# risingwavelabs/risingwave

Measured on NVIDIA H100. Metric: Nexmark q7/q8-shaped streaming HashJoin input rows/s, higher is better.
Workload: dtype int64

## Files before the change

__graft_entry__.py:

```python
import os
import subprocess
import sys

ROOT = os.path.dirname(os.path.abspath(__file__))
CSRC = os.path.join(ROOT, "risingwave_b200", "csrc")
BUILD = os.path.join(ROOT, "build")
LIB = os.path.join(ROOT, "risingwave_b200", "librwgpu.so")
NVCC = os.environ.get("NVCC", "/usr/local/cuda/bin/nvcc")
NVCC_FLAGS = ["-gencode", "arch=compute_90a,code=sm_90a", "-lineinfo", "-O3", "-std=c++17",
              "-Xcompiler", "-fPIC", "-Xcompiler", "-Wall"]
SOURCES = ["api.cu", "agg.cu", "join.cu", "shuffle.cu", "chain.cu"]


def _newer(target, deps):
    if not os.path.exists(target):
        return True
    t = os.path.getmtime(target)
    return any(os.path.getmtime(d) > t for d in deps)


def build_e2e_caller() -> str:
    os.makedirs(BUILD, exist_ok=True)
    e2e_src = os.path.join(ROOT, "tools", "e2e_caller.cc")
    e2e_bin = os.path.join(BUILD, "e2e_caller")
    if _newer(e2e_bin, [e2e_src, os.path.join(ROOT, "include", "rwgpu.h"), LIB]):
        subprocess.check_call(["g++", "-std=c++17", "-O2", "-Wall", "-I" + os.path.join(ROOT, "include"), "-I/usr/local/cuda/include", e2e_src,
                               "-o", e2e_bin, "-L" + os.path.join(ROOT, "risingwave_b200"), "-lrwgpu", "-L/usr/local/cuda/lib64", "-lcudart",
                               "-Wl,-rpath,$ORIGIN/../risingwave_b200", "-Wl,-rpath,/usr/local/cuda/lib64"])
    return e2e_bin


def build(verbose: bool = False) -> None:
    os.makedirs(BUILD, exist_ok=True)
    headers = [os.path.join(CSRC, f) for f in os.listdir(CSRC) if f.endswith((".cuh", ".h"))]
    headers.append(os.path.join(ROOT, "include", "rwgpu.h"))
    objs = []
    for src in SOURCES:
        s = os.path.join(CSRC, src)
        o = os.path.join(BUILD, src.replace(".cu", ".o"))
        objs.append(o)
        if _newer(o, [s] + headers):
            cmd = [NVCC] + NVCC_FLAGS + (["-Xptxas", "-v"] if verbose else []) + ["-c", s, "-o", o]
            subprocess.check_call(cmd)
    if _newer(LIB, objs):
        subprocess.check_call([NVCC] + NVCC_FLAGS[:2] + ["-shared", "-o", LIB] + objs + ["-lcudart"])
    subprocess.check_call(["make", "-s", "-C", os.path.join(ROOT, "oracle")])
    kat_src = os.path.join(ROOT, "tests", "cpp", "test_executor_kats.cc")
    kat_bin = os.path.join(BUILD, "test_executor_kats")
    if _newer(kat_bin, [kat_src, os.path.join(ROOT, "include", "rwgpu_executor.hpp"), LIB]):
        subprocess.check_call(["g++", "-std=c++17", "-O1", "-Wall", "-I" + os.path.join(ROOT, "include"), kat_src, "-o", kat_bin,
                               "-L" + os.path.join(ROOT, "risingwave_b200"), "-lrwgpu", "-Wl,-rpath,$ORIGIN/../risingwave_b200"])
    wm_src = os.path.join(ROOT, "tests", "cpp", "test_watermarks.cc")
    wm_bin = os.path.join(BUILD, "test_watermarks")
    if _newer(wm_bin, [wm_src, os.path.join(ROOT, "include", "rwgpu_executor.hpp"), LIB]):
        subprocess.check_call(["g++", "-std=c++17", "-O1", "-Wall", "-I" + os.path.join(ROOT, "include"), wm_src, "-o", wm_bin,
                               "-L" + os.path.join(ROOT, "risingwave_b200"), "-lrwgpu", "-Wl,-rpath,$ORIGIN/../risingwave_b200"])
    build_e2e_caller()
    sys.path.insert(0, ROOT)
    import risingwave_b200
    from risingwave_b200 import abi
    lib = abi.load_library()
    for sym in abi.ABI_SYMBOLS:
        getattr(lib, sym)


def smoke() -> None:
    sys.path.insert(0, ROOT)
    sys.path.insert(0, os.path.join(ROOT, "tests"))
    import ctypes
    import numpy as np
    from risingwave_b200.executor import Backend
    from risingwave_b200.stream_chunk import net_multiset
    import helpers
    cuda = Backend.cuda()
    oracle = Backend(ctypes.CDLL(os.path.join(ROOT, "oracle", "_build", "liboracle.so")), "rwo_")
    rng = np.random.default_rng(0)
    from risingwave_b200 import abi
    cfg = {"schema": "III", "group_keys": [0], "agg_calls": ["(count:int8)", "(sum:int8 $1:int8)", "(max:int8 $2:int8)"],
           "append_only": True, "row_count_index": 0}
    outs = []
    for be in (cuda, oracle):
        tx, ex = helpers.make_agg(be, cfg)
        res = []
        r2 = np.random.default_rng(1)
        for epoch in range(2):
            ex.apply_chunk(helpers.rand_chunk(r2, 4096, [abi.T_INT64] * 3, key_cols=(0,), key_range=300))
            res.append(net_multiset(ex.flush_data(epoch + 1)))
        outs.append(res)
    assert outs[0] == outs[1], "HashAgg smoke: CUDA result differs from oracle"
    print("smoke: HashAgg parity ok")
    try:
        kat = [k for k in helpers.load_golden("hash_join_kats.json") if k["name"] == "test_streaming_hash_inner_join"][0]
        helpers.run_join_kat(cuda, kat, exact=False)
        print("smoke: HashJoin golden ok")
    except abi.RwError as e:
        if e.code != abi.RW_ERR_UNSUPPORTED:
            raise
        print("smoke: HashJoin not built yet")


if __name__ == "__main__":
    build(verbose="-v" in sys.argv)
    print("build ok:", LIB)
```

risingwave_b200/csrc/join.cu:

```cuda
#include <algorithm>
#include <chrono>
#include <cstdio>
#include <cstdlib>
#include <memory>
#include <mutex>
#include <thread>

#include <cub/device/device_radix_sort.cuh>
#include <cub/device/device_scan.cuh>

#include "common.cuh"

namespace rw {

#define J_EMPTY 0x8000000000000000ull
#define J_NIL 0x7fffffffu
#define J_DEAD 0x80000000u
#define J_MAX_OUT (2 * RW_MAX_COLS)
#define J_HDR 16
#define W_EMPTY 0x7fffffffull
#define W_COUNT_ONE (1ull << 33)
#define W_IL_LIVE (1ull << 31)
#define W_IL_DEAD (2ull << 31)
#define W_IL_MASK (3ull << 31)
__device__ __host__ __forceinline__ uint32_t W_head(uint64_t W) { return (uint32_t)(W & 0x7fffffffull); }
__device__ __host__ __forceinline__ uint32_t W_istate(uint64_t W) { return (uint32_t)((W >> 31) & 3ull); }
__device__ __host__ __forceinline__ uint32_t W_count(uint64_t W) { return (uint32_t)(W >> 33); }

#define JERR_DOUBLE_DELETE 1u
#define JERR_OUT_CAPACITY 2u
#define JERR_APPEND_ONLY_MULTI 4u
#define JERR_STORE_CAPACITY 8u
#define JERR_BAD_COUNT 16u

struct JoinPlanDev {
  int T;
  int n_keys;
  int key_col[2][RW_MAX_KEYS];
  int null_safe[RW_MAX_KEYS];
  int n_cols[2];
  int col_type[2][RW_MAX_COLS];
  int col_width[2][RW_MAX_COLS];
  int col_off[2][RW_MAX_COLS];
  int stride[2];
  int bhdr;
  int bstride[2];
  int n_pk[2];
  int pk_col[2][RW_MAX_COLS];
  int n_out;
  int out_type[J_MAX_OUT];
  int out_width[J_MAX_OUT];
  int n_map[2];
  int map_in[2][J_MAX_OUT];
  int map_out[2][J_MAX_OUT];
  int need_degree[2];
  int append_only_optimize;
  int cond_cmp, cond_lhs, cond_rhs;
  int single_key, KW, SW;
  int strict;
};

struct JoinSideDev {
  uint8_t* recs;
  uint8_t* buckets;
  uint64_t cap;
  int stride;
  int bstride;
};

struct JoinStatus {
  unsigned long long out_rows;
  unsigned long long n_store;
  unsigned long long n_del;
  unsigned long long null_mask;
  unsigned long long n_keys[2];
  unsigned int err;
  unsigned int pad;
  unsigned long long n_in;
  unsigned long long log_next[2];
  unsigned long long n_dead[2];
  unsigned long long n_defer;
};

struct JoinOutDev {
  uint8_t* ops;
  uint8_t* vis;
  void* col[J_MAX_OUT];
  uint8_t* valid[J_MAX_OUT];
  int64_t capacity;
  const uint8_t* heap[2];
};

__device__ __host__ __forceinline__ bool jt_is_outer_side(int T, int S) { return T == RW_JOIN_FULL_OUTER || (T == RW_JOIN_LEFT_OUTER && S == 0) || (T == RW_JOIN_RIGHT_OUTER && S == 1); }
__device__ __host__ __forceinline__ bool jt_outer_side_null(int T, int S) { return T == RW_JOIN_FULL_OUTER || (T == RW_JOIN_LEFT_OUTER && S == 1) || (T == RW_JOIN_RIGHT_OUTER && S == 0); }
__device__ __host__ __forceinline__ bool jt_forward_exactly_once(int T, int S) { return ((T == RW_JOIN_LEFT_SEMI || T == RW_JOIN_LEFT_ANTI) && S == 0) || ((T == RW_JOIN_RIGHT_SEMI || T == RW_JOIN_RIGHT_ANTI) && S == 1); }
__device__ __host__ __forceinline__ bool jt_only_forward_matched_side(int T, int S) { return ((T == RW_JOIN_LEFT_SEMI || T == RW_JOIN_LEFT_ANTI) && S == 1) || ((T == RW_JOIN_RIGHT_SEMI || T == RW_JOIN_RIGHT_ANTI) && S == 0); }
__device__ __host__ __forceinline__ bool jt_is_semi(int T) { return T == RW_JOIN_LEFT_SEMI || T == RW_JOIN_RIGHT_SEMI; }
__device__ __host__ __forceinline__ bool jt_is_anti(int T) { return T == RW_JOIN_LEFT_ANTI || T == RW_JOIN_RIGHT_ANTI; }
__device__ __host__ __forceinline__ bool jt_forward_if_not_matched(int T, int S) { return (jt_is_anti(T) && jt_forward_exactly_once(T, S)) || jt_is_outer_side(T, S); }

struct RecHdr {
  uint32_t link, nullmask, seq, degree;
};
__device__ __forceinline__ uint8_t* rec_ptr(const JoinSideDev& s, uint32_t row) { return s.recs + (uint64_t)row * s.stride; }
__device__ __forceinline__ RecHdr* rec_hdr(const JoinSideDev& s, uint32_t row) { return (RecHdr*)rec_ptr(s, row); }

__device__ __forceinline__ uint64_t rec_key_word(const uint8_t* rec, int off, int width, int type) {
  ColRef cr;
  cr.data = rec + off;
  cr.valid_bits = nullptr;
  cr.valid_bytes = nullptr;
  cr.type = type;
  cr.width = width;
  return load_key_word(cr, 0);
}

__device__ __forceinline__ void prefetch_l2(const void* ptr) { asm volatile("prefetch.global.L2 [%0];" ::"l"(ptr)); }

__device__ __forceinline__ void copy_bytes(void* dst, const void* src, int width) {
  switch (width) {
    case 1: *(uint8_t*)dst = *(const uint8_t*)src; break;
    case 2: *(uint16_t*)dst = *(const uint16_t*)src; break;
    case 4: *(uint32_t*)dst = *(const uint32_t*)src; break;
    case 8: *(uint64_t*)dst = *(const uint64_t*)src; break;
    default: *(ulonglong2*)dst = *(const ulonglong2*)src; break;
  }
}

__device__ __forceinline__ bool chunk_key(const JoinPlanDev* p, int S, const DevChunk& ch, int64_t r, uint64_t* kw,
                                          uint32_t* nm) {
  uint32_t m = 0;
  bool never = false;
  for (int k = 0; k < p->n_keys; k++) {
    const ColRef& c = ch.cols[p->key_col[S][k]];
    if (col_is_null(c, r)) {
      m |= 1u << k;
      kw[k] = 0;
      if (!p->null_safe[k]) never = true;
    } else {
      kw[k] = load_key_word(c, r);
    }
  }
  *nm = m;
  return never;
}

__device__ __forceinline__ uint64_t key_hash(const JoinPlanDev* p, const uint64_t* kw, uint32_t nm) {
  uint64_t h = 0x9e3779b97f4a7c15ull ^ nm;
  for (int k = 0; k < p->n_keys; k++) h = mix64(h ^ kw[k]) + 0x9e3779b97f4a7c15ull;
  return h;
}

__device__ __forceinline__ uint64_t home64(uint64_t key, uint64_t mask) { return mix64(key) & mask & ~1ull; }

__device__ __forceinline__ uint8_t* bkt(const JoinSideDev& s, int64_t b) { return s.buckets + (uint64_t)b * s.bstride; }
__device__ __forceinline__ unsigned long long* bkt_W(const JoinSideDev& s, const JoinPlanDev* p, int64_t b) {
  return (unsigned long long*)(bkt(s, b) + p->KW * 8);
}
__device__ __forceinline__ uint8_t* bkt_inline(const JoinSideDev& s, const JoinPlanDev* p, int64_t b) { return bkt(s, b) + p->bhdr; }

__device__ __forceinline__ bool cas128(void* addr, ulonglong2 expect, ulonglong2 desired, ulonglong2* found) {
  unsigned long long o0, o1;
  asm volatile(
      "{\n .reg .b128 c, d, o;\n mov.b128 c, {%2, %3};\n mov.b128 d, {%4, %5};\n atom.global.cas.b128 o, [%6], c, d;\n mov.b128 {%0, %1}, o;\n}"
      : "=l"(o0), "=l"(o1)
      : "l"(expect.x), "l"(expect.y), "l"(desired.x), "l"(desired.y), "l"(addr)
      : "memory");
  found->x = o0;
  found->y = o1;
  return o0 == expect.x && o1 == expect.y;
}

__device__ __forceinline__ bool w_claim_inline(unsigned long long* Wp) {
  unsigned long long cur = __ldcg(Wp);
  while (W_istate(cur) != 1u) {
    const unsigned long long nw = ((cur & ~W_IL_MASK) | W_IL_LIVE) + W_COUNT_ONE;
    const unsigned long long old = atomicCAS(Wp, cur, nw);
    if (old == cur) return true;
    cur = old;
  }
  return false;
}
__device__ __forceinline__ uint32_t w_push_overflow(unsigned long long* Wp, uint32_t row) {
  unsigned long long cur = __ldcg(Wp);
  while (true) {
    const unsigned long long nw = ((cur & ~0x7fffffffull) | (unsigned long long)row) + W_COUNT_ONE;
// ... 1261 lines not shown
  d.cap = s.slot_cap;
  d.stride = s.stride;
  d.bstride = s.bstride;
  return d;
}

static int join_alloc_slots(rwgpu_join* h, int S, DevBuf& buf, uint64_t cap) {
  const int bs = h->side[S].bstride;
  RW_CUDA(buf.reserve((cap + 2) * (size_t)bs));
  join_init_slots_kernel<<<jgrid((int64_t)cap + 2, 256), 256, 0, h->stream>>>(buf.as<uint8_t>(), cap, bs, h->plan.KW, h->plan.single_key);
  RW_CUDA(cudaGetLastError());
  h->launches++;
  return RW_OK;
}

static int join_grow_store(rwgpu_join* h, int S, uint64_t rows) {
  JoinSideHost& s = h->side[S];
  if (h->uni) {
    if (rows >= 0x7ffffff0ull) return fail(RW_ERR_OOM, "join side exceeds 2^31 rows");
    int rc = RW_OK;
    if (rows > s.log.cap()) {
      rc = s.log.ensure(rows, h->last_st ? h->last_st : h->stream);
      s.row_cap = s.log.cap();
    }
    if (rc == RW_OK && !s.log.segs.empty() && rows + U_SEG_RECS > s.log.cap() && rows * 2 > s.log.cap()) s.log.prefetch();
    return rc;
  }
  if (rows <= s.row_cap) return RW_OK;
  if (rows >= 0x7ffffff0ull) return fail(RW_ERR_OOM, "join side exceeds 2^31 rows");
  size_t free_b = 0, total_b = 0;
  cudaMemGetInfo(&free_b, &total_b);
  const size_t va_limit = std::min<size_t>((size_t)0x7ffffff0ull * (size_t)s.stride, std::max<size_t>(total_b, (size_t)1 << 30));
  RW_CUDA(cudaDeviceSynchronize());
  const uint64_t live_rows = std::min<uint64_t>(s.n_rows, s.row_cap);
  cudaError_t e = s.recs.ensure((size_t)rows * (size_t)s.stride, (size_t)live_rows * (size_t)s.stride, va_limit, h->stream);
  if (e != cudaSuccess) return fail(RW_ERR_OOM, std::string("join record store: ") + cudaGetErrorString(e));
  s.row_cap = std::min<uint64_t>(s.recs.bytes() / (size_t)s.stride, 0x7ffffff0ull);
  return RW_OK;
}

static int join_grow_slots(rwgpu_join* h, int S, uint64_t need_keys) {
  JoinSideHost& s = h->side[S];
  if (need_keys * 2 <= s.slot_cap) return RW_OK;
  uint64_t ncap = s.slot_cap;
  while (ncap < need_keys * 4) ncap <<= 1;
  DevBuf nb;
  int rc = join_alloc_slots(h, S, nb, ncap);
  if (rc != RW_OK) return rc;
  join_rehash_kernel<<<jgrid((int64_t)s.slot_cap + 2, 256), 256, 0, h->stream>>>(s.slots.as<uint8_t>(), s.slot_cap, nb.as<uint8_t>(), ncap,
                                                                                  s.bstride, h->plan.KW, h->plan.single_key, h->plan.n_keys);
  RW_CUDA(cudaGetLastError());
  h->launches++;
  RW_CUDA(cudaStreamSynchronize(h->stream));
  s.slots = std::move(nb);
  s.slot_cap = ncap;
  return RW_OK;
}

static int join_ensure_scratch(rwgpu_join* h, int64_t n) {
  if (n > h->scratch_rows) {
    int64_t cap = std::max<int64_t>(n, 4096);
    RW_CUDA(h->sk.reserve((size_t)cap * 8));
    RW_CUDA(h->sk_alt.reserve((size_t)cap * 8));
    RW_CUDA(h->packed.reserve((size_t)cap * 8));
    RW_CUDA(h->offs.reserve((size_t)cap * 8));
    RW_CUDA(h->mslot.reserve((size_t)cap * 8));
    uint64_t g = 1024;
    while (g < (uint64_t)cap * 2) g <<= 1;
    RW_CUDA(h->gtable.reserve(g * 4));
    h->gcap = g;
    size_t b1 = 0, b2 = 0;
    cub::DeviceScan::ExclusiveSum(nullptr, b1, (uint64_t*)nullptr, (uint64_t*)nullptr, (int)cap);
    cub::DoubleBuffer<uint64_t> db((uint64_t*)nullptr, (uint64_t*)nullptr);
    cub::DeviceRadixSort::SortKeys(nullptr, b2, db, (int)cap);
    h->cub_bytes = std::max(b1, b2) + 256;
    RW_CUDA(h->cub_tmp.reserve(h->cub_bytes));
    h->scratch_rows = cap;
  }
  return RW_OK;
}

static int join_ensure_out(rwgpu_join* h, int64_t rows, cudaStream_t st, int64_t keep = 0) {
  if (rows <= h->os().out_cap) return RW_OK;
  int64_t cap = std::max<int64_t>(rows + rows / 4, 4096);
  RW_CUDA(cudaDeviceSynchronize());
  auto grow = [&](DevBuf& b, size_t elt, bool fill_one) -> int {
    DevBuf nb;
    RW_CUDA(nb.reserve((size_t)cap * elt));
    if (fill_one) RW_CUDA(cudaMemset(nb.p, 1, (size_t)cap * elt));
    if (keep > 0 && b.p) RW_CUDA(cudaMemcpy(nb.p, b.p, (size_t)keep * elt, cudaMemcpyDeviceToDevice));
    b = std::move(nb);
    return RW_OK;
  };
  int rc = grow(h->os().out_ops, 1, false);
  if (rc != RW_OK) return rc;
  rc = grow(h->os().out_vis, 1, false);
  if (rc != RW_OK) return rc;
  RW_CUDA(h->os().out_visbits.reserve((size_t)((cap + 63) / 64) * 8));
  for (size_t k = 0; k < h->out_types.size(); k++) {
    rc = grow(h->os().out_col[k], (size_t)type_width(h->out_types[k]), false);
    if (rc != RW_OK) return rc;
    rc = grow(h->os().out_valid[k], 1, true);
    if (rc != RW_OK) return rc;
    RW_CUDA(h->os().out_bits[k].reserve((size_t)((cap + 63) / 64) * 8));
  }
  if (keep == 0) h->os().valid_dirty = 0;
  h->os().out_cap = cap;
  return RW_OK;
}

static int join_clean_valid(rwgpu_join* h, cudaStream_t st) {
  for (size_t k = 0; k < h->out_types.size(); k++)
    if ((h->os().valid_dirty >> k) & 1) RW_CUDA(cudaMemsetAsync(h->os().out_valid[k].p, 1, (size_t)h->os().out_cap, st));
  h->os().valid_dirty = 0;
  return RW_OK;
}

static JoinOutDev out_dev(rwgpu_join* h) {
  JoinOutDev o;
  memset(&o, 0, sizeof(o));
  o.ops = h->os().out_ops.as<uint8_t>();
  o.vis = h->os().out_vis.as<uint8_t>();
  for (size_t k = 0; k < h->out_types.size(); k++) { o.col[k] = h->os().out_col[k].p; o.valid[k] = h->os().out_valid[k].as<uint8_t>(); }
  o.capacity = h->os().out_cap;
  o.heap[0] = h->var_heap[0].as<uint8_t>();
  o.heap[1] = h->var_heap[1].as<uint8_t>();
  return o;
}

__global__ void join_status_to_host_kernel(JoinStatus* src, JoinStatus* dst_host, unsigned long long tag, int reset) {
  join_status_publish(src, dst_host, tag, reset);
}
static int join_read_status(rwgpu_join* h, cudaStream_t st, JoinStatus* out, int reset = 1, unsigned long long tag = 0) {
  JoinStatus* host = h->status_host.as<JoinStatus>();
  if (tag) {
    RW_CUDA(cudaStreamSynchronize(st));
    if (*(volatile unsigned long long*)(host + 1) == tag) {
      memcpy(out, host, sizeof(JoinStatus));
      return RW_OK;
    }
  }
  join_status_to_host_kernel<<<1, 1, 0, st>>>(h->status.as<JoinStatus>(), host, 0ull, reset);
  RW_CUDA(cudaGetLastError());
  h->launches++;
  RW_CUDA(cudaStreamSynchronize(st));
  memcpy(out, host, sizeof(JoinStatus));
  return RW_OK;
}

static int join_check_err(rwgpu_join* h, const JoinStatus& s, cudaStream_t st) {
  if (!s.err) return RW_OK;
  unsigned int e = s.err;
  cudaMemsetAsync(&h->status.as<JoinStatus>()->err, 0, sizeof(unsigned int), st);
  if (e & JERR_DOUBLE_DELETE) return fail(RW_ERR_INCONSISTENT, "removing a join state entry but it is not in the cache");
  if (e & JERR_APPEND_ONLY_MULTI) return fail(RW_ERR_INCONSISTENT, "append-only optimisation: more than one matched row");
  if (e & JERR_STORE_CAPACITY) return fail(RW_ERR_CUDA, "internal: join record store capacity");
  if (e & JERR_BAD_COUNT) return fail(RW_ERR_INVALID, "device row count out of range");
  return fail(RW_ERR_CUDA, "internal: join output capacity");
}

static UniDev uni_dev(rwgpu_join* h) {
  UniDev t;
  t.buckets = h->uni_buckets.as<uint8_t>();
  t.cap = h->uni_cap;
  unsigned long long* ctr = h->uni_counters.as<unsigned long long>();
  for (int s = 0; s < 2; s++) {
    t.log[s] = h->side[s].log.table.as<uint8_t*>();
    t.log_cap[s] = h->side[s].log.cap();
    t.pools[s] = h->side[s].pools.as<uint2>();
    t.log_next[s] = ctr + s;
    t.n_dead[s] = ctr + 2 + s;
  }
  t.is = h->uni_is;
  return t;
}

static int uni_alloc_buckets(rwgpu_join* h, DevBuf& buf, uint64_t cap) {
  RW_CUDA(buf.reserve((cap + 2) * 64));
  uni_init_kernel<<<jgrid((int64_t)cap + 2, 256), 256, 0, h->stream>>>(buf.as<uint8_t>(), 0, cap + 2);
  RW_CUDA(cudaGetLastError());
  h->launches++;
  return RW_OK;
}

static int uni_grow_table(rwgpu_join* h, uint64_t need_keys) {
  if (need_keys * 2 <= h->uni_cap) return RW_OK;
  if (h->uni_keys_exact * 2 <= h->uni_cap && need_keys * 10 <= h->uni_cap * 9) return RW_OK;
  uint64_t ncap = h->uni_cap;
  while (ncap < need_keys * 4) ncap <<= 1;
  RW_CUDA(cudaDeviceSynchronize());
  DevBuf nb;
  int rc = uni_alloc_buckets(h, nb, ncap);
  if (rc != RW_OK) return rc;
  uni_rehash_kernel<<<jgrid((int64_t)h->uni_cap + 2, 256), 256, 0, h->stream>>>(h->uni_buckets.as<uint8_t>(), h->uni_cap, nb.as<uint8_t>(), ncap);
  RW_CUDA(cudaGetLastError());
  h->launches++;
  RW_CUDA(cudaStreamSynchronize(h->stream));
  h->uni_buckets = std::move(nb);
  h->uni_cap = ncap;
  return RW_OK;
}

static int uni_compact(rwgpu_join* h, int s) {
  JoinSideHost& sd = h->side[s];
  RW_CUDA(cudaDeviceSynchronize());
  SegLog fresh;
  const uint64_t live_upper = sd.n_rows > h->uni_dead[s] ? sd.n_rows - h->uni_dead[s] : 0;
  int rc = fresh.ensure(std::max<uint64_t>(live_upper, 1), h->stream);
  if (rc != RW_OK) { set_error(""); return RW_OK; }
  unsigned long long* ctr = h->uni_counters.as<unsigned long long>();
  RW_CUDA(cudaMemsetAsync(ctr + 4, 0, 8, h->stream));
  uni_compact_kernel<<<jgrid((int64_t)h->uni_cap + 2, 256), 256, 0, h->stream>>>(uni_dev(h), s, fresh.table.as<uint8_t*>(), ctr + 4);
  RW_CUDA(cudaGetLastError());
  h->launches++;
  unsigned long long live = 0;
  RW_CUDA(cudaMemcpyAsync(&live, ctr + 4, 8, cudaMemcpyDeviceToHost, h->stream));
  RW_CUDA(cudaStreamSynchronize(h->stream));
  std::swap(sd.log.segs, fresh.segs);
  {
    DevBuf t2 = std::move(sd.log.table);
    sd.log.table = std::move(fresh.table);
    fresh.table = std::move(t2);
  }
  sd.row_cap = sd.log.cap();
  sd.n_rows = live;
  h->uni_dead[s] = 0;
  const unsigned long long zero = 0;
  RW_CUDA(cudaMemcpyAsync(ctr + s, &live, 8, cudaMemcpyHostToDevice, h->stream));
  RW_CUDA(cudaMemcpyAsync(ctr + 2 + s, &zero, 8, cudaMemcpyHostToDevice, h->stream));
  RW_CUDA(cudaMemsetAsync(sd.pools.p, 0, sd.pools.bytes, h->stream));
  RW_CUDA(cudaStreamSynchronize(h->stream));
  h->compactions++;
  return RW_OK;
}

static int join_order(rwgpu_join* h, cudaStream_t st) {
  if (h->last_st && h->last_st != st) {
    if (!h->order_ev) RW_CUDA(cudaEventCreateWithFlags(&h->order_ev, cudaEventDisableTiming));
    RW_CUDA(cudaEventRecord(h->order_ev, h->last_st));
    RW_CUDA(cudaStreamWaitEvent(st, h->order_ev, 0));
  }
  h->last_st = st;
  return RW_OK;
}

static int uni_tail_grid(int64_t n) {
  static int max_blocks = 0;
  if (!max_blocks) {
    int dev = 0, sms = 0, per_sm = 0;
    cudaGetDevice(&dev);
    cudaDeviceGetAttribute(&sms, cudaDevAttrMultiProcessorCount, dev);
    int a = 0, b = 0;
    cudaOccupancyMaxActiveBlocksPerMultiprocessor(&a, uni_tail_kernel<false>, 256, 0);
    cudaOccupancyMaxActiveBlocksPerMultiprocessor(&b, uni_tail_kernel<true>, 256, 0);
    per_sm = std::max(1, std::min(std::min(a, b), 3));
    max_blocks = std::max(1, sms * per_sm);
  }
  return (int)std::max<int64_t>(1, std::min<int64_t>((n + 255) / 256, max_blocks));
}

static int uni_launch_main(rwgpu_join* h, const JoinPending& pd, bool probe_only, unsigned long long tag) {
  UniDev t = uni_dev(h);
  const JoinPlanDev* pdev = h->plan_dev.as<JoinPlanDev>();
  JoinStatus* ds = h->status.as<JoinStatus>();
  int S = pd.S;
  const bool is_row = S == h->uni_is;
  JoinOutDev od = out_dev(h);
  UniWork wk;
  wk.entry = h->uni_wk_entry.as<UniDefer>();
  wk.mask = h->uni_wk_mask.as<uint8_t>();
  W8Plan w = h->w8[S];
  h->prof.begin(pd.st);
  if (pd.plain) {
    PlainChunk pc;
    pc.ops = pd.ch.ops;
    for (int c = 0; c < 4; c++) pc.c[c] = c < w.n_u ? (const unsigned long long*)pd.ch.cols[c].data : nullptr;
    pc.key = (const unsigned long long*)pd.ch.cols[w.key_col].data;
    pc.n = pd.ch.n;
    pc.n_dev = pd.ch.n_dev;
    UniOwn own;
    own.log = t.log[S];
    own.log_cap = t.log_cap[S];
    own.pools = t.pools[S];
    own.log_next = t.log_next[S];
    PlainOut po;
    po.ops = od.ops;
    po.vis = od.vis;
    for (int c = 0; c < 4; c++) {
      po.ucol[c] = (!pd.alias_u && c < w.n_u && w.u_out[c] >= 0) ? (unsigned long long*)od.col[w.u_out[c]] : nullptr;
      po.mcol[c] = (c < w.n_m && w.m_out[c] >= 0) ? (unsigned long long*)od.col[w.m_out[c]] : nullptr;
    }
    po.capacity = od.capacity;
    auto hot = probe_only ? (is_row ? uni_hot_kernel<true, true> : uni_hot_kernel<true, false>)
                          : (is_row ? uni_hot_kernel<false, true> : uni_hot_kernel<false, false>);
    hot<<<pd.grid, JF_BLOCK, 0, pd.st>>>(pc, t.buckets, t.cap, own, po, wk, ds, pd.seq_base, pd.out_base, pd.pool_chunk);
  } else {
    if (probe_only) uni_slow_kernel<true><<<jgrid(pd.ch.n, 256), 256, 0, pd.st>>>(pdev, w, S, pd.ch, t, od, ds, pd.seq_base, pd.out_base);
    else uni_slow_kernel<false><<<jgrid(pd.ch.n, 256), 256, 0, pd.st>>>(pdev, w, S, pd.ch, t, od, ds, pd.seq_base, pd.out_base);
  }
  h->prof.end(pd.st);
  RW_CUDA(cudaGetLastError());
  DevChunk chv = pd.ch;
  uint64_t seq_base = pd.seq_base;
  int64_t out_base = pd.out_base;
  JoinStatus* slot = (JoinStatus*)(h->status_host.as<uint8_t>() + 512 * pd.set);
  int reset = 3;
  unsigned int* done = (unsigned int*)(h->uni_counters.as<unsigned long long>() + 6);
  const int tg = uni_tail_grid(pd.ch.n);
  if (probe_only) uni_tail_kernel<true><<<tg, 256, 0, pd.st>>>(pdev, w, S, chv, t, od, wk, ds, seq_base, out_base, slot, tag, reset, done);
  else uni_tail_kernel<false><<<tg, 256, 0, pd.st>>>(pdev, w, S, chv, t, od, wk, ds, seq_base, out_base, slot, tag, reset, done);
  RW_CUDA(cudaGetLastError());
  h->launches += 2;
  return RW_OK;
}

static int join_plain_chunk(DevChunk* ch, bool device_count, cudaStream_t st, bool* plain) {
  *plain = ch->vis_bits == nullptr;
  for (int c = 0; c < ch->n_cols && *plain; c++)
    *plain = !ch->cols[c].valid_bits && !ch->cols[c].valid_bytes && (((uintptr_t)ch->cols[c].data & 7) == 0);
  if (!ch->n_dev || (device_count && *plain)) return RW_OK;
  int64_t nh = 0;
  RW_CUDA(cudaMemcpyAsync(&nh, ch->n_dev, sizeof(nh), cudaMemcpyDeviceToHost, st));
  RW_CUDA(cudaStreamSynchronize(st));
  if (nh < 0 || nh > ch->n) return fail(RW_ERR_INVALID, "device row count out of range");
  ch->n = nh;
  ch->n_dev = nullptr;
  return RW_OK;
}

static double uni_now_ms() { return std::chrono::duration<double, std::milli>(std::chrono::steady_clock::now().time_since_epoch()).count(); }
static const bool uni_trace = getenv("RWGPU_TRACE") != nullptr;

static int uni_enqueue(rwgpu_join* h, int S, const DevChunk& ch_in, cudaStream_t st, int64_t out_base, bool alias_ok, JoinPending* pd) {
  const double tr0 = uni_trace ? uni_now_ms() : 0.0;
  DevChunk ch = ch_in;
  bool plain_cols;
  int rc = join_plain_chunk(&ch, true, st, &plain_cols);
  if (rc != RW_OK) return rc;
  const bool counted = ch.n_dev != nullptr;
  const int64_t n = ch.n;
  JoinSideHost& own = h->side[S];
  const int grid = (int)std::max<int64_t>(1, std::min<int64_t>((n + 63) / 64, U_MAX_GRID));
  uint32_t pool_chunk = 32;
  while (pool_chunk < 256 && (int64_t)pool_chunk * grid * 8 < 4 * n) pool_chunk <<= 1;
  const uint64_t id_slack = (uint64_t)grid * 8 * pool_chunk;
  rc = join_grow_store(h, S, own.n_rows + (uint64_t)n + id_slack);
  if (rc != RW_OK) return rc;
  rc = uni_grow_table(h, h->uni_keys + (uint64_t)n);
  if (rc != RW_OK) return rc;
  rc = join_ensure_out(h, out_base + n + std::max<int64_t>(n / 2, 4096), st, out_base);
  if (rc != RW_OK) return rc;
  if (plain_cols && n > h->uni_wk_cap) {
    RW_CUDA(cudaDeviceSynchronize());
    const int64_t cap = n + n / 4 + 64;
    RW_CUDA(h->uni_wk_entry.reserve((size_t)cap * sizeof(UniDefer)));
    RW_CUDA(h->uni_wk_mask.reserve((size_t)(cap + 7) / 8 + 16));
    h->uni_wk_cap = cap;
  }
  rc = join_order(h, st);
  if (rc != RW_OK) return rc;
  const double tr1 = uni_trace ? uni_now_ms() : 0.0;
  pd->S = S;
  pd->ch = ch;
  pd->st = st;
  pd->out_base = out_base;
  pd->set = h->cur;
  pd->plain = plain_cols;
  pd->counted = counted;
  pd->alias_u = alias_ok && plain_cols && !counted && out_base == 0 && h->var_in[S].empty();
  pd->grid = grid;
  pd->pool_chunk = pool_chunk;
  pd->seq_base = h->seq;
  pd->tag = ++h->status_tag;
  pd->ids_before = own.n_rows;
  pd->keys_before = h->uni_keys;
  h->seq += (uint64_t)n;
  own.n_rows += (uint64_t)n + id_slack;
  h->uni_keys += (uint64_t)n;
  rc = uni_launch_main(h, *pd, false, pd->tag);
  if (rc != RW_OK) return rc;
  if (!h->pend_ev[pd->set]) RW_CUDA(cudaEventCreateWithFlags(&h->pend_ev[pd->set], cudaEventDisableTiming));
  RW_CUDA(cudaEventRecord(h->pend_ev[pd->set], st));
  if (uni_trace)
    fprintf(stderr, "  [uni_enqueue S=%d n=%lld set=%d] grow/ensure %.3f ms, launch %.3f ms (log segs %zu/%zu, cap %llu keys<=%llu)\n", S, (long long)n,
            pd->set, tr1 - tr0, uni_now_ms() - tr1, h->side[0].log.segs.size(), h->side[1].log.segs.size(), (unsigned long long)h->uni_cap,
            (unsigned long long)h->uni_keys);
  return RW_OK;
}

static int uni_finish(rwgpu_join* h, const JoinPending& pd, int64_t* out_rows, unsigned long long* null_mask, bool* aliased = nullptr) {
  cudaStream_t st = pd.st;
  JoinStatus* ds = h->status.as<JoinStatus>();
  JoinStatus* slot = (JoinStatus*)(h->status_host.as<uint8_t>() + 512 * pd.set);
  JoinStatus hs;
  const double tr0 = uni_trace ? uni_now_ms() : 0.0;
  RW_CUDA(cudaEventSynchronize(h->pend_ev[pd.set]));
  const double tr1 = uni_trace ? uni_now_ms() : 0.0;
  int rc;
  if (*(volatile unsigned long long*)(slot + 1) != pd.tag) return fail(RW_ERR_CUDA, "join status block was not published");
  memcpy(&hs, slot, sizeof(JoinStatus));
  unsigned int err = hs.err;
  const unsigned long long first_null = hs.null_mask;
  const bool first_match = hs.pad != 0;
  const unsigned long long first_del = hs.n_del;
  const bool redone = (hs.err & JERR_OUT_CAPACITY) != 0;
  if (redone) {
    const int64_t extras = (int64_t)hs.out_rows, n = pd.ch.n;
    RW_CUDA(cudaMemsetAsync(&ds->err, 0, 4, st));
    rc = join_ensure_out(h, pd.out_base + n + extras + (int64_t)pd.grid * 8 * U_XCHUNK, st, pd.out_base);
    if (rc != RW_OK) return rc;
    const unsigned long long tag2 = ++h->status_tag;
    rc = uni_launch_main(h, pd, true, tag2);
    if (rc != RW_OK) return rc;
    RW_CUDA(cudaStreamSynchronize(st));
    if (*(volatile unsigned long long*)(slot + 1) != tag2) return fail(RW_ERR_CUDA, "join status block was not published");
    memcpy(&hs, slot, sizeof(JoinStatus));
    err = (err & ~JERR_OUT_CAPACITY) | hs.err;
    hs.null_mask |= first_null & ~(1ull << 63);
    hs.pad = hs.pad || first_match;
    hs.n_del = first_del;
  }
  for (int s = 0; s < 2; s++) h->uni_dead[s] = hs.n_dead[s];
  {
    JoinSideHost& own = h->side[pd.S];
    const uint64_t n = (uint64_t)pd.ch.n, slack = (uint64_t)pd.grid * 8 * pd.pool_chunk;
    const uint64_t rows_now = hs.log_next[pd.S] + (own.n_rows - (pd.ids_before + n + slack));
    const uint64_t keys_now = hs.n_keys[0] + (h->uni_keys - (pd.keys_before + n));
    for (int i = 0; i < h->n_pending; i++) {
      h->pending[i].ids_before += rows_now - own.n_rows;
      h->pending[i].keys_before += keys_now - h->uni_keys;
    }
    own.n_rows = rows_now;
    h->uni_keys = keys_now;
    h->uni_keys_exact = hs.n_keys[0];
  }
  hs.err = err;
  rc = join_check_err(h, hs, st);
  if (rc != RW_OK) return rc;
  const int64_t n_eff = pd.counted ? (int64_t)hs.n_in : pd.ch.n;
  *out_rows = (hs.pad != 0 || hs.out_rows) ? n_eff + (int64_t)hs.out_rows : 0;
  h->call_null_mask |= hs.null_mask;
  *null_mask = h->call_null_mask;
  h->os().valid_dirty |= hs.null_mask & ((1ull << 63) - 1);
  if (hs.n_del) h->call_had_deletes = true;
  const bool alias = pd.alias_u && !redone && hs.out_rows == 0 && !h->call_had_deletes;
  if (pd.alias_u && !alias && *out_rows > 0) {
    const W8Plan& w = h->w8[pd.S];
    for (int c = 0; c < w.n_u; c++)
      if (w.u_out[c] >= 0)
        RW_CUDA(cudaMemcpyAsync(h->os().out_col[w.u_out[c]].p, pd.ch.cols[c].data, (size_t)pd.ch.n * 8, cudaMemcpyDeviceToDevice, st));
  }
  if (aliased) *aliased = alias;
  if (uni_trace)
    fprintf(stderr, "  [uni_finish S=%d set=%d] wait %.3f ms, rest %.3f ms (redo %d, extras %llu, n_del %llu, out %lld)\n", pd.S, pd.set, tr1 - tr0,
            uni_now_ms() - tr1, (int)redone, (unsigned long long)hs.out_rows,
            (unsigned long long)hs.n_del, (long long)*out_rows);
  return RW_OK;
}

static int join_push_dev_uni(rwgpu_join* h, int S, const DevChunk& ch_in, cudaStream_t st, int64_t out_base, int64_t* out_rows,
                             unsigned long long* null_mask, bool* aliased) {
  if (h->n_pending) return fail(RW_ERR_INVALID, "collect the outstanding asynchronous pushes first");
  JoinPending pd;
  int rc = uni_enqueue(h, S, ch_in, st, out_base, aliased != nullptr, &pd);
  if (rc != RW_OK) return rc;
  return uni_finish(h, pd, out_rows, null_mask, aliased);
}

static int join_push_dev(rwgpu_join* h, int S, const DevChunk& ch_in, cudaStream_t st, int64_t out_base, int64_t* out_rows,
                         unsigned long long* null_mask, bool* aliased = nullptr) {
  *out_rows = 0;
  if (aliased) *aliased = false;
  DevChunk ch = ch_in;
  if (ch.n <= 0) return RW_OK;
  if (ch.n >= (1ll << 31)) return fail(RW_ERR_INVALID, "chunk too large");
  if (h->uni) return join_push_dev_uni(h, S, ch_in, st, out_base, out_rows, null_mask, aliased);
  bool plain_cols;
  int rc = join_plain_chunk(&ch, false, st, &plain_cols);
  if (rc != RW_OK) return rc;
  if (ch.n == 0) return RW_OK;
  const int64_t n = ch.n;
  JoinSideHost& own = h->side[S];
  static const bool trace = getenv("RWGPU_TRACE") != nullptr;
  auto now = []() { return std::chrono::duration<double, std::milli>(std::chrono::steady_clock::now().time_since_epoch()).count(); };
  const double tt0 = now();
  const uint64_t cap0 = own.slot_cap, rcap0 = own.row_cap;
  rc = join_grow_store(h, S, own.n_rows + (uint64_t)n);
  if (rc != RW_OK) return rc;
  rc = join_grow_slots(h, S, own.keys_upper + (uint64_t)n);
  if (rc != RW_OK) return rc;
  if (trace)
    fprintf(stderr, "  [push_dev S=%d n=%lld] grow %.3f ms (slot_cap %llu->%llu, row_cap %llu->%llu, n_rows %llu keys %llu)\n", S, (long long)n,
            now() - tt0, (unsigned long long)cap0, (unsigned long long)own.slot_cap, (unsigned long long)rcap0,
            (unsigned long long)own.row_cap, (unsigned long long)own.n_rows, (unsigned long long)own.keys_upper);
  JoinStatus* ds = h->status.as<JoinStatus>();
  const JoinPlanDev* pd = h->plan_dev.as<JoinPlanDev>();
  const uint64_t seq_base = h->seq;
  h->seq += (uint64_t)n;
  JoinStatus hs;
  if (h->fast_inner) {
    const bool use_w8 = h->w8_ok[S] && plain_cols;
    if (use_w8) {
      rc = join_ensure_out(h, out_base + n + std::max<int64_t>(n / 2, 4096), st, out_base);
      if (rc != RW_OK) return rc;
      const int grid = jgrid(n, JF_BLOCK);
      auto launch = [&](bool probe_only, uint32_t store_base) {
        if (probe_only)
          join_inner_w8p_kernel<true><<<grid, JF_BLOCK, 0, st>>>(pd, h->w8[S], S, ch, side_dev(h, S), side_dev(h, 1 - S), out_dev(h), ds,
                                                                  store_base, seq_base, out_base);
        else
          join_inner_w8p_kernel<false><<<grid, JF_BLOCK, 0, st>>>(pd, h->w8[S], S, ch, side_dev(h, S), side_dev(h, 1 - S), out_dev(h), ds,
                                                                   store_base, seq_base, out_base);
      };
      h->prof.begin(st);
      launch(false, (uint32_t)own.n_rows);
      h->prof.end(st);
      const unsigned long long tag = ++h->status_tag;
      join_inner_delete_kernel<<<jgrid(n, 256), 256, 0, st>>>(pd, S, ch, side_dev(h, S), ds, seq_base, h->status_host.as<JoinStatus>(), tag, 3);
      RW_CUDA(cudaGetLastError());
      h->launches += 2;
      rc = join_read_status(h, st, &hs, 3, tag);
      if (rc != RW_OK) return rc;
      const uint64_t stored = hs.n_store, keys = hs.n_keys[S];
      if (hs.n_del) h->call_had_deletes = true;
      unsigned int err = hs.err;
      if (hs.err & JERR_OUT_CAPACITY) {
        const int64_t extras = (int64_t)hs.out_rows;
        RW_CUDA(cudaMemsetAsync(&ds->out_rows, 0, 8, st));
        RW_CUDA(cudaMemsetAsync(&ds->err, 0, 4, st));
        RW_CUDA(cudaStreamSynchronize(st));
        rc = join_ensure_out(h, out_base + n + extras, st, out_base);
        if (rc != RW_OK) return rc;
        launch(true, 0u);
        RW_CUDA(cudaGetLastError());
        h->launches++;
        rc = join_read_status(h, st, &hs, 3);
        if (rc != RW_OK) return rc;
        err = (err & ~JERR_OUT_CAPACITY) | hs.err;
      }
      own.n_rows += stored;
      own.keys_upper = keys;
      const bool any_match = hs.pad != 0;
      hs.err = err;
      rc = join_check_err(h, hs, st);
      if (rc != RW_OK) return rc;
      *out_rows = (any_match || hs.out_rows) ? n + (int64_t)hs.out_rows : 0;
    } else {
      rc = join_ensure_out(h, out_base + std::max<int64_t>(2 * n, 4096), st, out_base);
      if (rc != RW_OK) return rc;
      h->out_rows_cumulative = true;
      h->call_vis_stale = true;
      const int64_t tiles = (n + JF_BLOCK * JF_R - 1) / (JF_BLOCK * JF_R);
      const int grid = (int)std::max<int64_t>(1, std::min<int64_t>(tiles, RW_SMS * 8));
      h->prof.begin(st);
      join_inner_fused_kernel<false><<<grid, JF_BLOCK, 0, st>>>(pd, S, ch, side_dev(h, S), side_dev(h, 1 - S), out_dev(h), ds,
                                                                  (uint32_t)own.n_rows, seq_base);
      h->prof.end(st);
      join_inner_delete_kernel<<<jgrid(n, 256), 256, 0, st>>>(pd, S, ch, side_dev(h, S), ds, seq_base, nullptr, 0ull, 0);
// ... 1134 lines not shown
```

risingwave_b200/csrc/join_uni.cuh:

```cuda
#pragma once
#include <cooperative_groups.h>

namespace rw {

#define U_NIL 0x7fffffffu
#define U_XCHUNK 64
#define U_MAX_GRID (RW_SMS * 8)

#define U_SEG_SHIFT 22
#define U_SEG_RECS (1u << U_SEG_SHIFT)
#define U_MAX_SEGS 512
struct UniDev {
  uint8_t* buckets;
  uint64_t cap;
  uint8_t* const* log[2];
  uint64_t log_cap[2];
  uint2* pools[2];
  unsigned long long* log_next[2];
  unsigned long long* n_dead[2];
  int is;
};

struct UniRec {
  uint32_t link, nullmask;
// ... 563 lines not shown
      const unsigned long long want = (warp_defer ? 1ull : 0ull) | (warp_sentinel ? 2ull : 0ull);
      if (want && (__ldcg(&st->n_defer) & want) != want) atomicOr(&st->n_defer, want);
    }
    if (!PROBE_ONLY && new_keys) atomicAdd(&st->n_keys[0], (unsigned long long)new_keys);
    if (!PROBE_ONLY && n_del) atomicAdd(&st->n_del, (unsigned long long)n_del);
  }
}

template <bool PROBE_ONLY>
__device__ __forceinline__ void uni_deferred_body(const JoinPlanDev* __restrict__ p, const W8Plan& w, int S, const DevChunk& ch, const UniDev& t,
                                                  const JoinOutDev& o, const UniWork& wk, JoinStatus* st, uint64_t seq_base, int64_t out_base) {
  const int64_t n_rows = chunk_rows(ch);
  unsigned new_keys = 0;
  bool any_match = false, any_hole = false;
  for (int64_t r = blockIdx.x * (int64_t)blockDim.x + threadIdx.x; r < n_rows; r += (int64_t)gridDim.x * blockDim.x) {
    if (!((wk.mask[r >> 3] >> (r & 7)) & 1u)) continue;
    const UniDefer e = wk.entry[r];
    const uint8_t op = ch.ops[r];
    const int64_t pos = out_base + r;
    if (e.cnt == 0u) {
      uni_row_generic<PROBE_ONLY>(p, w, S, ch, r, op, t, o, st, seq_base + (uint64_t)r, pos, out_base + n_rows, new_keys, any_match, any_hole);
    } else {
      any_match = true;
      o.vis[pos] = 1;
      const bool ins = (op == RW_OP_INSERT || op == RW_OP_UPDATE_INSERT);
      uni_emit_matches(t, w, S, ch, r, ins ? RW_OP_INSERT : RW_OP_DELETE, e.b, e.cnt, o, st, pos, e.xpos);
    }
  }
  if (any_hole) atomicOr(&st->null_mask, 1ull << 63);
  if (any_match) st->pad = 1u;
  if (!PROBE_ONLY && new_keys) atomicAdd(&st->n_keys[0], (unsigned long long)new_keys);
}

__device__ __forceinline__ bool uni_pk_equal(const JoinPlanDev* p, int S, const uint64_t* c, uint32_t nmask, const DevChunk& ch, int64_t r) {
  for (int i = 0; i < p->n_pk[S]; i++) {
    const int k = p->pk_col[S][i];
    const bool n1 = (nmask >> k) & 1u, n2 = col_is_null(ch.cols[k], r);
    if (n1 != n2) return false;
    if (n1) continue;
    if (c[k] != ((const uint64_t*)ch.cols[k].data)[r]) return false;
  }
  return true;
}

__device__ __forceinline__ void uni_delete_body(const JoinPlanDev* __restrict__ p, int S, const DevChunk& ch, const UniDev& t, JoinStatus* st,
                                                uint64_t seq_base, int sentinel_mode) {
  const int64_t n_rows = chunk_rows(ch);
  const uint64_t SEQ56 = (1ull << 56) - 1;
  unsigned int dead_log = 0;
  const int64_t r_first = sentinel_mode == 2 ? (int64_t)threadIdx.x : blockIdx.x * (int64_t)blockDim.x + threadIdx.x;
  const int64_t r_step = sentinel_mode == 2 ? (int64_t)blockDim.x : (int64_t)gridDim.x * blockDim.x;
  for (int64_t r = r_first; r < n_rows; r += r_step) {
    const uint8_t op = ch.ops[r];
    if (!row_visible(ch, r, op) || !(op == RW_OP_DELETE || op == RW_OP_UPDATE_DELETE)) continue;
    const ColRef& kc = ch.cols[p->key_col[S][0]];
    const bool knull = col_is_null(kc, r);
    if (knull && !p->null_safe[0]) continue;
    const uint64_t key = knull ? 0ull : ((const uint64_t*)kc.data)[r];
    if (sentinel_mode && ((!knull && key == J_EMPTY) != (sentinel_mode == 2))) continue;
    const int64_t b = uni_find(t, key, knull);
    bool found = false;
    while (b >= 0 && !found) {
      int best_kind = 0;
      uint32_t best_id = U_NIL;
      uint64_t best_seq = 0;
      auto consider = [&](int kind, uint32_t id, uint64_t seq, const uint64_t* c, uint32_t nmask) {
        const uint64_t d = (seq - seq_base) & SEQ56;
        if (d < (uint64_t)n_rows && d >= (uint64_t)r) return;
        if (!uni_pk_equal(p, S, c, nmask, ch, r)) return;
        const uint64_t rank = d < (uint64_t)n_rows ? (1ull << 60) + d : (seq & SEQ56);
        if (best_kind == 0 || rank > best_seq) { best_kind = kind; best_id = id; best_seq = rank; }
      };
      uint32_t m;
      if (S == t.is) {
        const unsigned long long WI = __ldcg(ub_WI(t, b));
        if (W_istate(WI) == 1u) {
          const unsigned long long ih = __ldcg(ub_IH(t, b));
          uint64_t c[4];
          const ulonglong2 c01 = __ldcg((const ulonglong2*)(ub(t, b) + 32)), c23 = __ldcg((const ulonglong2*)(ub(t, b) + 48));
          c[0] = c01.x; c[1] = c01.y; c[2] = c23.x; c[3] = c23.y;
          consider(1, 0u, ih >> 8, c, (uint32_t)(ih & 0xffull));
        }
        m = W_head(WI);
      } else {
        m = __ldcg(ub_chead(t, b));
      }
      while (m != U_NIL) {
        const UniRec* rec = urec(t, S, m);
        const ulonglong2 h0 = __ldcg((const ulonglong2*)rec);
        const uint32_t lk = (uint32_t)h0.x;
        if (!(lk & J_DEAD)) {
          uint64_t c[4];
          const ulonglong2 c01 = __ldcg((const ulonglong2*)rec + 1), c23 = __ldcg((const ulonglong2*)rec + 2);
          c[0] = c01.x; c[1] = c01.y; c[2] = c23.x; c[3] = c23.y;
          consider(2, m, h0.y, c, (uint32_t)(h0.x >> 32));
        }
        m = lk & 0x7fffffffu;
      }
      if (best_kind == 0) break;
      if (best_kind == 1) {
        unsigned long long* Wp = ub_WI(t, b);
        unsigned long long cur = __ldcg(Wp);
        while (W_istate(cur) == 1u) {
          const unsigned long long old = atomicCAS(Wp, cur, ((cur & ~W_IL_MASK) | W_IL_DEAD) - W_COUNT_ONE);
          if (old == cur) { found = true; break; }
          cur = old;
        }
      } else {
        const uint32_t old = atomicOr(&urec(t, S, best_id)->link, J_DEAD);
        if (!(old & J_DEAD)) {
          if (S == t.is) atomicAdd(ub_WI(t, b), 0ull - W_COUNT_ONE);
          else atomicSub(ub_ccount(t, b), 1u);
          dead_log++;
          found = true;
        }
      }
    }
    if (!found && p->strict) atomicOr(&st->err, JERR_DOUBLE_DELETE);
  }
  if (dead_log) atomicAdd(t.n_dead[S], (unsigned long long)dead_log);
}

template <bool PROBE_ONLY>
__global__ void __launch_bounds__(256) uni_tail_kernel(const JoinPlanDev* __restrict__ p, W8Plan w, int S, DevChunk ch, UniDev t, JoinOutDev o, UniWork wk,
                                                       JoinStatus* st, uint64_t seq_base, int64_t out_base, JoinStatus* status_host,
                                                       unsigned long long tag, int reset, unsigned int* done) {
  __shared__ bool s_last;
  const unsigned long long defer_flags = *(volatile unsigned long long*)&st->n_defer;
  const bool has_del = !PROBE_ONLY && *(volatile unsigned long long*)&st->n_del != 0ull;
  const bool split = has_del && (defer_flags & 2ull) != 0ull;
  if (defer_flags) uni_deferred_body<PROBE_ONLY>(p, w, S, ch, t, o, wk, st, seq_base, out_base);
  if (has_del) uni_delete_body(p, S, ch, t, st, seq_base, split ? 1 : 0);
  __syncthreads();
  if (threadIdx.x == 0) {
    __threadfence();
    s_last = atomicAdd(done, 1u) == gridDim.x - 1;
  }
  __syncthreads();
  if (!s_last) return;
  __threadfence();
  if (split) {
    uni_delete_body(p, S, ch, t, st, seq_base, 2);
    __threadfence();
    __syncthreads();
  }
  if (threadIdx.x == 0) {
    done[0] = 0u;
    st->log_next[0] = *(volatile unsigned long long*)t.log_next[0]; st->log_next[1] = *(volatile unsigned long long*)t.log_next[1];
    st->n_dead[0] = *(volatile unsigned long long*)t.n_dead[0]; st->n_dead[1] = *(volatile unsigned long long*)t.n_dead[1];
    join_status_publish(st, status_host, tag, reset);
  }
}

__global__ void __launch_bounds__(256) uni_clean_kernel(UniDev t, int side, long long wm) {
  unsigned int dead = 0;
  for (uint64_t b = blockIdx.x * (uint64_t)blockDim.x + threadIdx.x; b < t.cap + 2; b += (uint64_t)gridDim.x * blockDim.x) {
    if (b == t.cap) continue;
    const unsigned long long key = *(const unsigned long long*)ub(t, (int64_t)b);
    if (b < t.cap && key == J_EMPTY) continue;
    const long long kv = b == t.cap + 1 ? (long long)J_EMPTY : (long long)key;
    if (kv >= wm) continue;
    if (side == t.is) {
      unsigned long long* Wp = ub_WI(t, (int64_t)b);
      const unsigned long long W = *Wp;
      const uint32_t cnt = W_count(W);
      if (cnt) dead += cnt - (W_istate(W) == 1u ? 1u : 0u);
      *Wp = W_EMPTY | (W_istate(W) ? W_IL_DEAD : 0ull);
    } else {
      dead += *ub_ccount(t, (int64_t)b);
      *ub_chead(t, (int64_t)b) = U_NIL;
      *ub_ccount(t, (int64_t)b) = 0u;
    }
  }
  for (int d = 16; d > 0; d >>= 1) dead += __shfl_xor_sync(0xffffffffu, dead, d);
  if (lane_id() == 0 && dead) atomicAdd(t.n_dead[side], (unsigned long long)dead);
}

__global__ void uni_status_kernel(UniDev t, JoinStatus* st, JoinStatus* status_host, unsigned long long tag, int reset) {
  st->log_next[0] = *t.log_next[0]; st->log_next[1] = *t.log_next[1];
  st->n_dead[0] = *t.n_dead[0]; st->n_dead[1] = *t.n_dead[1];
  join_status_publish(st, status_host, tag, reset);
}

__global__ void uni_rehash_kernel(const uint8_t* ob, uint64_t ocap, uint8_t* nb, uint64_t ncap) {
  for (uint64_t i = blockIdx.x * (uint64_t)blockDim.x + threadIdx.x; i < ocap + 2; i += (uint64_t)gridDim.x * blockDim.x) {
    const ulonglong2* s = (const ulonglong2*)(ob + i * 64);
    uint64_t dst;
    if (i >= ocap) {
      dst = ncap + (i - ocap);
    } else {
      const uint64_t key = s[0].x;
      if (key == J_EMPTY) continue;
      const uint64_t mask = ncap - 1;
      uint64_t idx = uhome(key, mask);
      while (atomicCAS((unsigned long long*)(nb + idx * 64), (unsigned long long)J_EMPTY, (unsigned long long)key) != J_EMPTY) idx = (idx + 1) & mask;
      dst = idx;
    }
    ulonglong2* d = (ulonglong2*)(nb + dst * 64);
    const ulonglong2 s0 = s[0];
    ((unsigned long long*)d)[1] = s0.y;
    if (i >= ocap) ((unsigned long long*)d)[0] = s0.x;
    d[1] = s[1]; d[2] = s[2]; d[3] = s[3];
  }
}

__global__ void uni_compact_kernel(UniDev t, int side, uint8_t* const* new_log, unsigned long long* new_next) {
  const int lane = lane_id();
  for (uint64_t i0 = (blockIdx.x * (uint64_t)blockDim.x + threadIdx.x) & ~31ull; i0 < t.cap + 2; i0 += (uint64_t)gridDim.x * blockDim.x) {
    const uint64_t i = i0 + lane;
    uint32_t live = 0, head = U_NIL;
    bool has = false;
    if (i < t.cap + 2) {
      const unsigned long long key = __ldcg((const unsigned long long*)ub(t, (int64_t)i));
      has = key != J_EMPTY || i >= t.cap;
      if (has) {
        head = side == t.is ? W_head(__ldcg(ub_WI(t, (int64_t)i))) : __ldcg(ub_chead(t, (int64_t)i));
        for (uint32_t m = head; m != U_NIL;) {
          const uint32_t lk = __ldcg(&urec(t, side, m)->link);
          if (!(lk & J_DEAD)) live++;
          m = lk & 0x7fffffffu;
        }
      }
    }
    uint32_t incl = live;
    for (int d = 1; d < 32; d <<= 1) {
      const uint32_t v = __shfl_up_sync(0xffffffffu, incl, d);
      if (lane >= d) incl += v;
    }
    const uint32_t total = __shfl_sync(0xffffffffu, incl, 31);
    unsigned long long base = 0;
    if (lane == 31 && total) base = atomicAdd(new_next, (unsigned long long)total);
    base = __shfl_sync(0xffffffffu, base, 31);
    if (!has) continue;
    uint32_t nid = (uint32_t)base + (incl - live);
    uint32_t new_head = U_NIL;
    UniRec* prev = nullptr;
    for (uint32_t m = head; m != U_NIL;) {
      const UniRec* rec = urec(t, side, m);
      const uint32_t lk = rec->link;
      if (!(lk & J_DEAD)) {
        UniRec* d = (UniRec*)useg_rec(new_log, nid);
        *d = *rec;
        d->link = U_NIL;
        if (prev) prev->link = nid; else new_head = nid;
        prev = d;
        nid++;
      }
      m = lk & 0x7fffffffu;
    }
    if (head != U_NIL) {
      if (side == t.is) {
        unsigned long long* Wp = ub_WI(t, (int64_t)i);
        *Wp = (*Wp & ~0x7fffffffull) | (unsigned long long)new_head;
      } else {
        *ub_chead(t, (int64_t)i) = new_head;
      }
    }
  }
}

}
```

Before: 5.301 billion.

## Launch join tail kernel conditionally from device via tail launch

Replaces the unconditional host launch of the join tail grid with a one-warp launcher kernel. The launcher reads the deferred-row and delete counts on device and only then tail-launches the full tail grid through dynamic parallelism, otherwise publishing status directly. This aims to skip the full tail grid when it has no work, at the cost of compiling join.cu with relocatable device code, linking cudadevrt, and adding a new error path if the device-side launch fails.

```diff
diff --git a/__graft_entry__.py b/__graft_entry__.py
--- a/__graft_entry__.py
+++ b/__graft_entry__.py
@@ -10,6 +10,7 @@
 NVCC_FLAGS = ["-gencode", "arch=compute_90a,code=sm_90a", "-lineinfo", "-O3", "-std=c++17",
               "-Xcompiler", "-fPIC", "-Xcompiler", "-Wall"]
 SOURCES = ["api.cu", "agg.cu", "join.cu", "shuffle.cu", "chain.cu"]
+RDC_SOURCES = {"join.cu"}
 
 
 def _newer(target, deps):
@@ -40,10 +41,10 @@
         o = os.path.join(BUILD, src.replace(".cu", ".o"))
         objs.append(o)
         if _newer(o, [s] + headers):
-            cmd = [NVCC] + NVCC_FLAGS + (["-Xptxas", "-v"] if verbose else []) + ["-c", s, "-o", o]
+            cmd = [NVCC] + NVCC_FLAGS + (["-Xptxas", "-v"] if verbose else []) + (["-rdc=true"] if src in RDC_SOURCES else []) + ["-c", s, "-o", o]
             subprocess.check_call(cmd)
     if _newer(LIB, objs):
-        subprocess.check_call([NVCC] + NVCC_FLAGS[:2] + ["-shared", "-o", LIB] + objs + ["-lcudart"])
+        subprocess.check_call([NVCC] + NVCC_FLAGS[:2] + ["-rdc=true", "-Xcompiler", "-fPIC", "-shared", "-o", LIB] + objs + ["-lcudadevrt", "-lcudart"])
     subprocess.check_call(["make", "-s", "-C", os.path.join(ROOT, "oracle")])
     kat_src = os.path.join(ROOT, "tests", "cpp", "test_executor_kats.cc")
     kat_bin = os.path.join(BUILD, "test_executor_kats")
diff --git a/risingwave_b200/csrc/join.cu b/risingwave_b200/csrc/join.cu
--- a/risingwave_b200/csrc/join.cu
+++ b/risingwave_b200/csrc/join.cu
@@ -32,6 +32,7 @@
 #define JERR_APPEND_ONLY_MULTI 4u
 #define JERR_STORE_CAPACITY 8u
 #define JERR_BAD_COUNT 16u
+#define JERR_TAIL_LAUNCH 32u
 
 struct JoinPlanDev {
   int T;
@@ -1599,6 +1600,7 @@
   if (!s.err) return RW_OK;
   unsigned int e = s.err;
   cudaMemsetAsync(&h->status.as<JoinStatus>()->err, 0, sizeof(unsigned int), st);
+  if (e & JERR_TAIL_LAUNCH) return fail(RW_ERR_CUDA, "internal: the device-side launch of the join tail kernel failed (deferred rows and deletes not applied)");
   if (e & JERR_DOUBLE_DELETE) return fail(RW_ERR_INCONSISTENT, "removing a join state entry but it is not in the cache");
   if (e & JERR_APPEND_ONLY_MULTI) return fail(RW_ERR_INCONSISTENT, "append-only optimisation: more than one matched row");
   if (e & JERR_STORE_CAPACITY) return fail(RW_ERR_CUDA, "internal: join record store capacity");
@@ -1754,8 +1756,8 @@
   int reset = 3;
   unsigned int* done = (unsigned int*)(h->uni_counters.as<unsigned long long>() + 6);
   const int tg = uni_tail_grid(pd.ch.n);
-  if (probe_only) uni_tail_kernel<true><<<tg, 256, 0, pd.st>>>(pdev, w, S, chv, t, od, wk, ds, seq_base, out_base, slot, tag, reset, done);
-  else uni_tail_kernel<false><<<tg, 256, 0, pd.st>>>(pdev, w, S, chv, t, od, wk, ds, seq_base, out_base, slot, tag, reset, done);
+  if (probe_only) uni_tail_launch_kernel<true><<<1, 32, 0, pd.st>>>(pdev, w, S, chv, t, od, wk, ds, seq_base, out_base, slot, tag, reset, done, tg);
+  else uni_tail_launch_kernel<false><<<1, 32, 0, pd.st>>>(pdev, w, S, chv, t, od, wk, ds, seq_base, out_base, slot, tag, reset, done, tg);
   RW_CUDA(cudaGetLastError());
   h->launches += 2;
   return RW_OK;
@@ -1850,7 +1852,7 @@
   const unsigned long long first_null = hs.null_mask;
   const bool first_match = hs.pad != 0;
   const unsigned long long first_del = hs.n_del;
-  const bool redone = (hs.err & JERR_OUT_CAPACITY) != 0;
+  const bool redone = (hs.err & JERR_OUT_CAPACITY) != 0 && !(hs.err & JERR_TAIL_LAUNCH);
   if (redone) {
     const int64_t extras = (int64_t)hs.out_rows, n = pd.ch.n;
     RW_CUDA(cudaMemsetAsync(&ds->err, 0, 4, st));
diff --git a/risingwave_b200/csrc/join_uni.cuh b/risingwave_b200/csrc/join_uni.cuh
--- a/risingwave_b200/csrc/join_uni.cuh
+++ b/risingwave_b200/csrc/join_uni.cuh
@@ -739,6 +739,24 @@
   }
 }
 
+template <bool PROBE_ONLY>
+__global__ void __launch_bounds__(32) uni_tail_launch_kernel(const JoinPlanDev* __restrict__ p, W8Plan w, int S, DevChunk ch, UniDev t, JoinOutDev o,
+                                                             UniWork wk, JoinStatus* st, uint64_t seq_base, int64_t out_base,
+                                                             JoinStatus* status_host, unsigned long long tag, int reset, unsigned int* done,
+                                                             int tail_grid) {
+  if (threadIdx.x != 0) return;
+  const bool has_del = !PROBE_ONLY && *(volatile unsigned long long*)&st->n_del != 0ull;
+  if (*(volatile unsigned long long*)&st->n_defer != 0ull || has_del) {
+    uni_tail_kernel<PROBE_ONLY><<<tail_grid, 256, 0, cudaStreamTailLaunch>>>(p, w, S, ch, t, o, wk, st, seq_base, out_base, status_host, tag,
+                                                                            reset, done);
+    if (cudaGetLastError() == cudaSuccess) return;
+    atomicOr(&st->err, JERR_TAIL_LAUNCH);
+  }
+  st->log_next[0] = *(volatile unsigned long long*)t.log_next[0]; st->log_next[1] = *(volatile unsigned long long*)t.log_next[1];
+  st->n_dead[0] = *(volatile unsigned long long*)t.n_dead[0]; st->n_dead[1] = *(volatile unsigned long long*)t.n_dead[1];
+  join_status_publish(st, status_host, tag, reset);
+}
+
 __global__ void __launch_bounds__(256) uni_clean_kernel(UniDev t, int side, long long wm) {
   unsigned int dead = 0;
   for (uint64_t b = blockIdx.x * (uint64_t)blockDim.x + threadIdx.x; b < t.cap + 2; b += (uint64_t)gridDim.x * blockDim.x) {
@@ -763,12 +781,6 @@
   if (lane_id() == 0 && dead) atomicAdd(t.n_dead[side], (unsigned long long)dead);
 }
 
-__global__ void uni_status_kernel(UniDev t, JoinStatus* st, JoinStatus* status_host, unsigned long long tag, int reset) {
-  st->log_next[0] = *t.log_next[0]; st->log_next[1] = *t.log_next[1];
-  st->n_dead[0] = *t.n_dead[0]; st->n_dead[1] = *t.n_dead[1];
-  join_status_publish(st, status_host, tag, reset);
-}
-
 __global__ void uni_rehash_kernel(const uint8_t* ob, uint64_t ocap, uint8_t* nb, uint64_t ncap) {
   for (uint64_t i = blockIdx.x * (uint64_t)blockDim.x + threadIdx.x; i < ocap + 2; i += (uint64_t)gridDim.x * blockDim.x) {
     const ulonglong2* s = (const ulonglong2*)(ob + i * 64);
```

Result: no change. 5.438 billion (median of 6 runs) (+2.6%).
